# eridgd/WCT-TF

Hardware: AMD Instinct MI355X
Metric: stylized frames/sec @512x512, 5-level relu5->1 pipeline, alpha=0.8 (higher is better)
Workload: dtype f16

## Files before the change

### wct_tf_amd/build.py

```python
import hashlib
import os
import subprocess
import sys
from concurrent.futures import ThreadPoolExecutor

HERE = os.path.dirname(os.path.abspath(__file__))
CSRC = os.path.join(HERE, 'csrc')
LIB = os.path.join(HERE, 'libwct_hip.so')
WCT_UNITS = ['stats_gemm.hip', 'eigh.hip', 'spectral.hip', 'wct.hip', 'mask.hip', 'style_swap.hip', 'warm.hip']
API_UNITS = ['api_ctx.hip', 'api_weights.hip', 'api_drivers.hip', 'api_ops.hip', 'api_stylize.hip', 'api_train.hip']
SOURCES = API_UNITS + ['conv.hip', 'conv_wino.hip', 'coral.hip', 'colors.hip', 'noise.hip', 'banded.hip', 'train.hip'] + WCT_UNITS


STAMP = LIB + '.src.sha256'
FLAGS = ['--offload-arch=gfx950', '-O3', '-std=c++17', '-fPIC', '-Wno-unused-value', '-Wno-unused-result']
FILE_FLAGS = {u: ['-fno-slp-vectorize'] for u in WCT_UNITS}


def source_digest():
    h = hashlib.sha256((' '.join(FLAGS) + repr(sorted(FILE_FLAGS.items()))).encode())
    deps = sorted(os.path.join(CSRC, f) for f in os.listdir(CSRC) if f.endswith(('.hip', '.h')))
    deps.append(os.path.join(os.path.dirname(HERE), 'include', 'wct_hip.h'))
    for d in deps:
        h.update(os.path.basename(d).encode())
        h.update(open(d, 'rb').read())
    return h.hexdigest()


def needs_build():
    if not (os.path.exists(LIB) and os.path.exists(STAMP)):
        return True
    return open(STAMP).read().strip() != source_digest()


def build(force=False, verbose=True):
    if not force and not needs_build():
        return LIB
    hipcc = os.environ.get('HIPCC', '/opt/rocm/bin/hipcc')
    objs = [os.path.join(CSRC, src.replace('.hip', '.o')) for src in SOURCES]

    def compile_unit(src, obj):
        cmd = [hipcc] + FLAGS + FILE_FLAGS.get(src, []) + ['-c', os.path.join(CSRC, src), '-o', obj]
        if verbose:
            print(' '.join(cmd), flush=True)
        subprocess.check_call(cmd)

    with ThreadPoolExecutor(min(16, len(SOURCES))) as pool:
        list(pool.map(compile_unit, SOURCES, objs))
    cmd = [hipcc, '--offload-arch=gfx950', '-shared', '-fPIC', '-o', LIB] + objs
    if verbose:
        print(' '.join(cmd), flush=True)
    subprocess.check_call(cmd)
    with open(STAMP, 'w') as f:
        f.write(source_digest() + '\n')
    return LIB


if __name__ == '__main__':
    build(force='--force' in sys.argv)
    print(LIB)
```

### wct_tf_amd/csrc/spectral.hip

```cpp
#include "wct_stages.h"

__device__ __forceinline__ bool pair_resolved(float dp, float dq, float e) { return e * e <= 0.25f * dp * dq; }

constexpr float SPECTRAL_NOISE_CUT = 2.f;
__device__ __forceinline__ float spectral_cut(const float* Am, int C, int tid, float* red) {
  float mn = 0.f;
  for (int i = tid; i < C; i += 256) mn = fminf(mn, Am[(size_t)i * C + i]);
  for (int o = 32; o > 0; o >>= 1) mn = fminf(mn, __shfl_xor(mn, o, 64));
  if ((tid & 63) == 0) red[tid >> 6] = mn;
  __syncthreads();
  mn = fminf(fminf(red[0], red[1]), fminf(red[2], red[3]));
  return fmaxf(1e-5f, -SPECTRAL_NOISE_CUT * mn);
}

__device__ __forceinline__ float spectral_entry(float dp, float dq, float e, bool diag, int kind, float shift, float cut) {
  const bool kp = dp > cut, kq = dq > cut;
  if (diag) return kp ? (kind == 0 ? 1.f / sqrtf(dp + shift) : sqrtf(dp + shift)) : 0.f;
  if (!kp && !kq) return 0.f;
  if (kp && kq) {
    if (!pair_resolved(dp, dq, e)) return 0.f;
    const float sa = sqrtf(dp + shift), sb = sqrtf(dq + shift);
    return kind == 0 ? -e / (sa * sb * (sa + sb)) : e / (sa + sb);
  }
  const float dk = kp ? dp : dq, dd = kp ? dq : dp;
// ... 163 lines not shown
  spectral_tile_load(t, Am, C, p0, q0, tid);
  __syncthreads();
  const int ty = tid >> 4, tx = tid & 15;
#pragma unroll
  for (int i = 0; i < 4; ++i) {
    const int pl = ty * 4 + i, p = p0 + pl, q = q0 + tx * 4;
    if (p >= C || q >= C) continue;
    const f32x4 av = *reinterpret_cast<const f32x4*>(Am + (size_t)p * C + q);
    const float dp = t.dp[pl];
    f32x4 g, n4 = {0.f, 0.f, 0.f, 0.f}, r4 = n4, p4 = n4;
#pragma unroll
    for (int j = 0; j < 4; ++j) {
      const float dk = t.dq[tx * 4 + j];
      const float em = 0.5f * (av[j] + t.mt[tx * 4 + j][pl]);
      g[j] = spectral_entry(dp, dk, a.correct ? em : 0.f, p == q + j, kind, a.shift, cut);
      if (a.second && p != q + j && dp > cut && dk > cut && pair_resolved(dp, dk, em)) {
        const float sp = sqrtf(dp + a.shift), sk = sqrtf(dk + a.shift);
        n4[j] = em / (sp + sk);
        r4[j] = em / sk;
        p4[j] = n4[j] / sk;
      }
    }
    const size_t o = (size_t)p * C + q;
    *reinterpret_cast<f32x4*>(a.G + m * cc + o) = g;
    if (a.second) {
      *reinterpret_cast<f32x4*>(a.N + m * cc + o) = n4;
      if (kind == 0) { *reinterpret_cast<f32x4*>(a.R + pair * cc + o) = r4; *reinterpret_cast<f32x4*>(a.Pm + pair * cc + o) = p4; }
    }
  }
}

__global__ __launch_bounds__(256) void spectral_add2_all_kernel(SpecAllArgs a) {
  __shared__ float dps[64], dqs[64];
  __shared__ float x1t[64][65], x2t[64][65];
  const int m = blockIdx.z, p0 = blockIdx.y * 64, q0 = blockIdx.x * 64, tid = threadIdx.x;
  if (skip_style_mat(m, a.shared_style)) return;
  const int C = a.C, kind = m & 1;
  const size_t cc = (size_t)C * C;
  const float* Am = a.A + m * cc;
  float* Gm = a.G + m * cc;
  const float* X2 = a.X2 + m * cc;
  const float* X1 = a.X1 + (size_t)(m >> 1) * cc;
  int near = 0;
  for (int i = tid; i < C; i += 256) {
    const float d = fabsf(Am[(size_t)i * C + i]);
    near |= (d > 3.3e-6f) & (d < 3e-5f);
  }
  if (__syncthreads_or(near)) return;
  __shared__ float cutred[4];
  const float cut = spectral_cut(Am, C, tid, cutred);
  if (tid < 64) dps[tid] = p0 + tid < C ? Am[(size_t)(p0 + tid) * C + p0 + tid] : 0.f;
  else if (tid < 128) dqs[tid - 64] = q0 + tid - 64 < C ? Am[(size_t)(q0 + tid - 64) * C + q0 + tid - 64] : 0.f;
  const int ty = tid >> 4, tx = tid & 15;
#pragma unroll
  for (int i = 0; i < 4; ++i) {
    const int r = q0 + ty * 4 + i, c = p0 + tx * 4;
    f32x4 v1 = {0.f, 0.f, 0.f, 0.f}, v2 = v1;
    if (r < C && c < C) {
      v2 = *reinterpret_cast<const f32x4*>(X2 + (size_t)r * C + c);
      if (kind == 0) v1 = *reinterpret_cast<const f32x4*>(X1 + (size_t)r * C + c);
    }
#pragma unroll
    for (int j = 0; j < 4; ++j) { x2t[ty * 4 + i][tx * 4 + j] = v2[j]; x1t[ty * 4 + i][tx * 4 + j] = v1[j]; }
  }
  __syncthreads();
#pragma unroll
  for (int i = 0; i < 4; ++i) {
    const int pl = ty * 4 + i, p = p0 + pl, q = q0 + tx * 4;
    if (p >= C || q >= C) continue;
    const size_t o = (size_t)p * C + q;
    const f32x4 x2 = *reinterpret_cast<const f32x4*>(X2 + o);
    f32x4 x1 = {0.f, 0.f, 0.f, 0.f};
    if (kind == 0) x1 = *reinterpret_cast<const f32x4*>(X1 + o);
    f32x4 g = *reinterpret_cast<const f32x4*>(Gm + o);
    const float dp = dps[pl];
#pragma unroll
    for (int j = 0; j < 4; ++j) {
      const float dq = dqs[tx * 4 + j];
      if (!(dp > cut && dq > cut)) continue;
      const float sp = sqrtf(dp + a.shift), sq = sqrtf(dq + a.shift);
      float l2;
      if (kind == 1) l2 = -0.5f * (x2[j] + x2t[tx * 4 + j][pl]) / (sp + sq);
      else l2 = (0.5f * (x1[j] + x1t[tx * 4 + j][pl]) + 0.25f * (sp + sq) * (x2[j] + x2t[tx * 4 + j][pl])) / (sp * sq * (sp + sq));
      g[j] += l2;
    }
    *reinterpret_cast<f32x4*>(Gm + o) = g;
  }
}

int launch_spectral_function(const float* A, const float* V, float* G, float* X, float* out, int C, int nbatch,
                                    size_t stride, size_t out_stride, int kind, float shift, hipStream_t s, float* scratch2) {
  const size_t cc = (size_t)C * C;
  const dim3 tiles(cdiv(C, 64), cdiv(C, 64), nbatch);
  hipLaunchKernelGGL(spectral_matrix_kernel, tiles, dim3(256), 0, s, A, G, C, stride, kind, shift, EIG_CORRECT);
  HIP_TRY(hipGetLastError());
  if (scratch2 && EIG_CORRECT >= 2) {
    float* N = scratch2; float* R = N + nbatch * cc; float* Pm = R + nbatch * cc; float* X1 = Pm + nbatch * cc; float* X2 = X1 + nbatch * cc;
    hipLaunchKernelGGL(spectral_prep2_kernel, tiles, dim3(256), 0, s, A, N, R, Pm, C, stride, kind, shift);
    HIP_TRY(hipGetLastError());
    GemmArgs a = {};
    a.A = kind == 1 ? N : Pm; a.lda = C; a.a_kmajor = 0; a.B = N; a.ldb = C; a.b_kmajor = 1; a.sA = a.sB = cc;
    a.M = C; a.N = C; a.K = C; a.ksplit = C; a.out32 = X2; a.ldo = C; a.s_out = cc;
    int rc2 = launch_gemm(a, 1, nbatch, s);
    if (rc2) return rc2;
    if (kind == 0) {
      a.A = R; a.out32 = X1;
      if ((rc2 = launch_gemm(a, 1, nbatch, s))) return rc2;
    }
    hipLaunchKernelGGL(spectral_add2_kernel, tiles, dim3(256), 0, s, A, G, X1, X2, C, stride, kind, shift);
    HIP_TRY(hipGetLastError());
  }
  GemmArgs g = {};
  g.A = V; g.lda = C; g.a_kmajor = 0; g.B = G; g.ldb = C; g.b_kmajor = 1; g.sA = g.sB = stride;
  g.M = C; g.N = C; g.K = C; g.ksplit = C; g.out32 = X; g.ldo = C; g.s_out = stride;
  int rc = launch_gemm(g, 1, nbatch, s);
  if (rc) return rc;
  GemmArgs h = {};
  h.A = X; h.lda = C; h.a_kmajor = 0; h.B = V; h.ldb = C; h.b_kmajor = 0; h.sA = h.sB = stride;
  h.M = C; h.N = C; h.K = C; h.ksplit = C; h.out32 = out; h.ldo = C; h.s_out = out_stride;
  return launch_gemm(h, 1, nbatch, s);
}

int launch_refresh(const WctCarve& w, int C, int P, int shared_style, hipStream_t s, bool always) {
  const size_t cc = (size_t)C * C;
  int rc;
  GemmArgs r1 = {};
  r1.A = w.A0; r1.lda = C; r1.a_kmajor = 0; r1.B = w.V; r1.ldb = C; r1.b_kmajor = 1; r1.sA = r1.sB = cc; r1.skip_shared = shared_style;
  r1.M = C; r1.N = C; r1.K = C; r1.ksplit = C; r1.out32 = w.X; r1.ldo = C; r1.s_out = cc;
  if (!always) { r1.mask_diag = w.A; r1.s_mask = cc; r1.mask_out = w.refresh; }
  if ((rc = launch_gemm(r1, 1, 2 * P, s))) return rc;
  GemmArgs r2 = {};
  r2.A = w.V; r2.lda = C; r2.a_kmajor = 1; r2.B = w.X; r2.ldb = C; r2.b_kmajor = 1; r2.sA = r2.sB = cc; r2.skip_shared = shared_style;
  r2.M = C; r2.N = C; r2.K = C; r2.ksplit = C; r2.out32 = w.A; r2.ldo = C; r2.s_out = cc;
  if (!always) r2.mask_in = w.refresh;
  rc = launch_gemm(r2, 1, 2 * P, s);
  return rc;
}

int launch_spectral_tail(const WctCarve& w, int C, int P, float alpha, int mode, float eps_in, int shared_style, int nwhite,
                                hipStream_t s) {
  int rc;
  const size_t cc = (size_t)C * C;
  const float shift = mode == WCT_MODE_NP ? (eps_in >= 0.f ? eps_in : 1e-5f) : 0.f;
  const int second = EIG_CORRECT >= 2;
  const dim3 tiles(cdiv(C, 64), cdiv(C, 64), 2 * P);
  if ((rc = launch_refresh(w, C, P, shared_style, s))) return rc;
  SpecAllArgs sa = {};
  sa.A = w.A; sa.G = w.G; sa.C = C; sa.shift = shift; sa.correct = EIG_CORRECT; sa.second = second; sa.shared_style = shared_style;
  sa.N = w.S2; float* X2 = sa.N + 2 * P * cc; sa.R = X2 + 2 * P * cc; sa.Pm = sa.R + P * cc; float* X1 = sa.Pm + P * cc;
  sa.X1 = X1; sa.X2 = X2;
  sa.mabs = w.mabs; sa.mean = w.mean; sa.bias = w.bias; sa.alpha = alpha; sa.mode = mode;
  hipLaunchKernelGGL(spectral_open_all_kernel, tiles, dim3(256), 0, s, sa);
  HIP_TRY(hipGetLastError());
  if (second) {
    GemmArgs a = {};
    a.A = sa.Pm; a.sA = cc; a.A_odd = sa.N + cc; a.sA_odd = 2 * cc; a.lda = C; a.a_kmajor = 0;
    a.B = sa.N; a.ldb = C; a.b_kmajor = 1; a.sB = cc; a.skip_shared = shared_style;
    a.M = C; a.N = C; a.K = C; a.ksplit = C; a.out32 = X2; a.ldo = C; a.s_out = cc;
    if ((rc = launch_gemm(a, 1, 2 * P, s))) return rc;
    GemmArgs b = {};
    b.A = sa.R; b.sA = cc; b.lda = C; b.a_kmajor = 0; b.B = sa.N; b.ldb = C; b.b_kmajor = 1; b.sB = 2 * cc;
    b.M = C; b.N = C; b.K = C; b.ksplit = C; b.out32 = X1; b.ldo = C; b.s_out = cc;
    if (nwhite > 0 && (rc = launch_gemm(b, 1, nwhite, s))) return rc;
    hipLaunchKernelGGL(spectral_add2_all_kernel, tiles, dim3(256), 0, s, sa);
    HIP_TRY(hipGetLastError());
  }
  GemmArgs g = {};
  g.A = w.V; g.lda = C; g.a_kmajor = 0; g.B = w.G; g.ldb = C; g.b_kmajor = 1; g.sA = g.sB = cc; g.skip_shared = shared_style;
  g.M = C; g.N = C; g.K = C; g.ksplit = C; g.out32 = w.X; g.ldo = C; g.s_out = cc;
  if ((rc = launch_gemm(g, 1, 2 * P, s))) return rc;
  GemmArgs h = {};
  h.A = w.X; h.lda = C; h.a_kmajor = 0; h.B = w.V; h.ldb = C; h.b_kmajor = 0; h.sA = h.sB = cc; h.skip_shared = shared_style;
  h.M = C; h.N = C; h.K = C; h.ksplit = C; h.out32 = w.Tw; h.ldo = C; h.s_out = cc;
  if ((rc = launch_gemm(h, 1, 2 * P, s))) return rc;
  return WCT_OK;
}
```

### wct_tf_amd/csrc/wct.hip

```cpp
#include "wct_stages.h"
#include "jacobi_dev.h"
#include <algorithm>
#include <type_traits>



template <int BC, int BP, typename Args = ApplyArgs>
__global__ __launch_bounds__(256, 2) void apply_f16x2_kernel(Args p) {
  constexpr bool SEGB = std::is_same<Args, ApplySegBatchArgs>::value;
  constexpr bool SEG = std::is_same<Args, ApplySegArgs>::value || SEGB;
  constexpr int TM = BC / 64, TN = BP / 64;
  constexpr int MI = BC * 4 / 256, XI = BP * 4 / 256;
  __shared__ __attribute__((aligned(16))) unsigned char lm[2][BC * 64];
  __shared__ __attribute__((aligned(16))) unsigned char lx[2][BP * 64];
  typedef unsigned int u32x4 __attribute__((ext_vector_type(4)));
  const int tid = threadIdx.x, lane = tid & 63, wave = tid >> 6;
  const int wm = wave >> 1, wn = wave & 1;
  const int pair = blockIdx.z;
  const int n0 = blockIdx.x * BP, c0 = blockIdx.y * BC;
  int seg0 = 0, N = p.N;
  [[maybe_unused]] int row0 = 0;
  if constexpr (SEGB) {
    const int f = seg_frame(p.fl[pair]), lab = seg_label(p.fl[pair]);
    const int first = p.seg_off[f * (WCT_MIX_MAX + 1) + lab];
// ... 77 lines not shown
#pragma unroll
    for (int ks = 0; ks < 2; ++ks) {
      const int chunk = ks * 2 + (lane >> 5);
      half8 ah[TM], al[TM], bh[TN], bl[TN];
#pragma unroll
      for (int i = 0; i < TM; ++i) {
        const int r = (wm * TM + i) * 32 + (lane & 31);
        const int off = (r * 4 + (chunk ^ ((r >> 2) & 3))) * 16;
        ah[i] = *reinterpret_cast<const half8*>(lm[0] + off);
        al[i] = *reinterpret_cast<const half8*>(lm[1] + off);
      }
#pragma unroll
      for (int j = 0; j < TN; ++j) {
        const int r = (wn * TN + j) * 32 + (lane & 31);
        const int off = (r * 4 + (chunk ^ ((r >> 2) & 3))) * 16;
        bh[j] = *reinterpret_cast<const half8*>(lx[0] + off);
        bl[j] = *reinterpret_cast<const half8*>(lx[1] + off);
      }
#pragma unroll
      for (int i = 0; i < TM; ++i)
#pragma unroll
        for (int j = 0; j < TN; ++j) {
          acc[i][j] = __builtin_amdgcn_mfma_f32_32x32x16_f16(al[i], bh[j], acc[i][j], 0, 0, 0);
          acc[i][j] = __builtin_amdgcn_mfma_f32_32x32x16_f16(ah[i], bl[j], acc[i][j], 0, 0, 0);
          acc[i][j] = __builtin_amdgcn_mfma_f32_32x32x16_f16(ah[i], bh[j], acc[i][j], 0, 0, 0);
        }
    }
    __syncthreads();
  }

  const float inv = 1.f / (sx * sM);
  const float* bias = p.bias + (size_t)pair * C;
  const int kgrp = lane >> 5;
  f32x4 bvs[TM][4];
#pragma unroll
  for (int i = 0; i < TM; ++i)
#pragma unroll
    for (int rq = 0; rq < 4; ++rq) {
      const int co = c0 + (wm * TM + i) * 32 + 8 * rq + 4 * kgrp;
      const f32x4 z = {0.f, 0.f, 0.f, 0.f};
      bvs[i][rq] = co < C ? *reinterpret_cast<const f32x4*>(bias + co) : z;
    }
  int dst[TN];
  if constexpr (SEG)
#pragma unroll
    for (int j = 0; j < TN; ++j) {
      const int n = n0 + (wn * TN + j) * 32 + (lane & 31);
      dst[j] = p.perm[seg0 + (n < N ? n : 0)];
      if constexpr (SEGB) dst[j] += row0;
    }
#pragma unroll
  for (int j = 0; j < TN; ++j) {
    const int n = n0 + (wn * TN + j) * 32 + (lane & 31);
    const bool n_ok = n < N;
    const size_t row = SEG ? (size_t)dst[j] * C : ((size_t)pair * N + (n_ok ? n : 0)) * C;
#pragma unroll
    for (int i = 0; i < TM; ++i) {
      const int cb = c0 + (wm * TM + i) * 32;
      unsigned pk[4][2];
#pragma unroll
      for (int rq = 0; rq < 4; ++rq) {
        const int co = cb + 8 * rq + 4 * kgrp;
        const f32x4 bv = bvs[i][rq];
        f32x4 v;
#pragma unroll
        for (int q = 0; q < 4; ++q) v[q] = acc[i][j][rq * 4 + q] * inv + bv[q];
        if (p.out32 && n_ok && co < C) *reinterpret_cast<f32x4*>(p.out32 + row + co) = v;
        typedef _Float16 h2 __attribute__((ext_vector_type(2)));
        h2 lo = {(half_t)v[0], (half_t)v[1]}, hi = {(half_t)v[2], (half_t)v[3]};
        pk[rq][0] = __builtin_bit_cast(unsigned, lo);
        pk[rq][1] = __builtin_bit_cast(unsigned, hi);
      }
      if (p.out16) {
#pragma unroll
        for (int m = 0; m < 2; ++m) {
          auto sxw = __builtin_amdgcn_permlane32_swap(pk[2 * m][0], pk[2 * m + 1][0], false, false);
          auto syw = __builtin_amdgcn_permlane32_swap(pk[2 * m][1], pk[2 * m + 1][1], false, false);
          u32x4 o = {sxw[0], syw[0], sxw[1], syw[1]};
          const int co = cb + 16 * m + 8 * kgrp;
          if (n_ok && co < C) *reinterpret_cast<u32x4*>(p.out16 + row + co) = o;
        }
      }
    }
  }
}

int launch_apply_seg(const ApplySegArgs& a, int nmax, int P, hipStream_t s) {
  const int C = a.C;
  if (C >= 128) hipLaunchKernelGGL((apply_f16x2_kernel<128, 128, ApplySegArgs>), dim3(cdiv(nmax, 128), cdiv(C, 128), P), dim3(256), 0, s, a);
  else hipLaunchKernelGGL((apply_f16x2_kernel<64, 128, ApplySegArgs>), dim3(cdiv(nmax, 128), cdiv(C, 64), P), dim3(256), 0, s, a);
  HIP_TRY(hipGetLastError());
  return WCT_OK;
}

int launch_apply_seg_batch(const ApplySegBatchArgs& a, int nmax, int P, hipStream_t s) {
  const int C = a.C;
  if (C >= 128) hipLaunchKernelGGL((apply_f16x2_kernel<128, 128, ApplySegBatchArgs>), dim3(cdiv(nmax, 128), cdiv(C, 128), P), dim3(256), 0, s, a);
  else hipLaunchKernelGGL((apply_f16x2_kernel<64, 128, ApplySegBatchArgs>), dim3(cdiv(nmax, 128), cdiv(C, 64), P), dim3(256), 0, s, a);
  HIP_TRY(hipGetLastError());
  return WCT_OK;
}

static int wct_nslab(int N) { int s = cdiv(N, 64); return s < 1 ? 1 : (s > 256 ? 256 : s); }

static void cov_split(int C, int Nmax, int P, int* nsplit, int* ksplit) {
  const int nt = C >= 128 ? cdiv(C, 128) : 1;
  const int tiles = nt * (nt + 1) / 2 * P;
  int want = 32 / tiles;
  if (want < 1) want = 1;
  int ks = cdiv(cdiv(Nmax, want), 32) * 32;
  if (ks < 256) ks = 256;
  *ksplit = ks;
  *nsplit = cdiv(Nmax, ks);
}

PairLayout pair_layout(int C, int Nc, int Ns) {
  PairLayout L;
  const int Nmax = Nc > Ns ? Nc : Ns;
  L.nslab = wct_nslab(Nmax);
  cov_split(C, Nmax, 1, &L.nsplit, &L.ksplit);
  return L;
}

WctCarve carve(void* base, int C, int P, const PairLayout& lay) {
  WctCarve w;
  w.nslab = lay.nslab; w.nsplit = lay.nsplit; w.ksplit = lay.ksplit;
  size_t off = 0;
  char* b = reinterpret_cast<char*>(base);
  auto take = [&](size_t bytes) { void* p = b ? b + off : nullptr; off += align_up(bytes); return p; };
  const size_t cc = (size_t)C * C * sizeof(float);
  w.mean = (float*)take((size_t)2 * P * C * sizeof(float));
  w.var = (float*)take((size_t)2 * P * C * sizeof(float));
  w.stat_partial = (float*)take((size_t)2 * P * w.nslab * C * sizeof(float));
  w.absmax = (float*)take((size_t)2 * P * w.nslab * sizeof(float));
  w.scale = (float*)take((size_t)2 * P * sizeof(float));
  w.cov_partial = (float*)take((size_t)2 * P * w.nsplit * cc);
  w.A = (float*)take(2 * P * cc);
  w.A0 = (float*)take(2 * P * cc);
  w.refresh = (int*)take((size_t)2 * P * sizeof(int));
  w.V = (float*)take(2 * P * cc);
  w.d = (float*)take((size_t)2 * P * C * sizeof(float));
  w.G = (float*)take(2 * P * cc);
  w.X = (float*)take(2 * P * cc);
  w.S2 = (float*)take(7 * P * cc);
  w.Tw = (float*)take(2 * P * cc);
  w.Tcs = w.Tw + (size_t)C * C;
  w.T = (float*)take(P * cc);
  w.M = (float*)take(P * cc);
  w.bias = (float*)take((size_t)P * C * sizeof(float));
  w.mabs = (unsigned*)take((size_t)P * sizeof(unsigned));
  w.jacobi_bytes = jacobi_workspace_bytes(C, 2 * P) + 4 * (1024 + 64 * sizeof(JacobiState));
  w.jacobi_ws = take(w.jacobi_bytes);
  w.mix = (float*)take((size_t)2 * C * sizeof(float));
  w.total = off;
  return w;
}

size_t wct_workspace_bytes(int C, int Nc, int Ns, int P) {
  const int Cw = C < 32 ? 32 : C;
  return carve(nullptr, Cw, P, pair_layout(Cw, Nc, Ns)).total;
}

int launch_blend(const WctCarve& w, int C, int P, float alpha, int shared_style, hipStream_t s) {
  const size_t cc = (size_t)C * C;
  GemmArgs g = {};
  g.A = w.Tcs; g.lda = C; g.a_kmajor = 0; g.B = w.Tw; g.ldb = C; g.b_kmajor = 1; g.sA = shared_style ? 0 : 2 * cc; g.sB = 2 * cc;
  g.M = C; g.N = C; g.K = C; g.ksplit = C; g.out32 = w.M; g.ldo = C; g.s_out = cc;
  g.blend = 1; g.alpha = alpha; g.mabs = w.mabs;
  return launch_gemm(g, 1, P, s);
}

int launch_apply(const WctCarve& w, const float* content, int Nc, int C, int P, half_t* out16, float* out32, hipStream_t s) {
  ApplyArgs a;
  a.x = content; a.N = Nc; a.C = C; a.mean = w.mean; a.M = w.M; a.bias = w.bias;
  a.xscale = w.scale; a.mabs = w.mabs; a.out16 = out16; a.out32 = out32;
  if (C >= 128) hipLaunchKernelGGL((apply_f16x2_kernel<128, 128>), dim3(cdiv(Nc, 128), cdiv(C, 128), P), dim3(256), 0, s, a);
  else hipLaunchKernelGGL((apply_f16x2_kernel<64, 128>), dim3(cdiv(Nc, 128), cdiv(C, 64), P), dim3(256), 0, s, a);
  HIP_TRY(hipGetLastError());
  return WCT_OK;
}

static int launch_blend_apply(const WctCarve& w, const float* content, int Nc, int C, int P, float alpha, int shared_style,
                              half_t* out16, float* out32, hipStream_t s) {
  int rc;
  if ((rc = launch_blend(w, C, P, alpha, shared_style, s))) return rc;
  return launch_apply(w, content, Nc, C, P, out16, out32, s);
}

WctStyleKey wct_style_key(int C, int Nc, int Ns) {
  const PairLayout L = pair_layout(std::max(C, 32), Nc, Ns);
  return WctStyleKey{L.nslab, L.nsplit, L.ksplit};
}
size_t wct_style_state_floats(int C) { return (size_t)2 * C + (size_t)C * C; }

template <typename Ref>
__global__ __launch_bounds__(256) void style_load_kernel(Ref r, float* mean, float* var, float* Tw, int C, int with_T) {
  const int k = blockIdx.y;
  const float* src = r.state[k];
  const size_t cc = (size_t)C * C, n = (size_t)2 * C + (with_T ? cc : 0), slot = (size_t)(2 * k + 1);
  for (size_t i = (blockIdx.x * (size_t)blockDim.x + threadIdx.x) * 4; i < n; i += (size_t)gridDim.x * blockDim.x * 4) {
    const f32x4 v = *reinterpret_cast<const f32x4*>(src + i);
    float* dst = i < (size_t)C ? mean + slot * C + i : (i < (size_t)2 * C ? var + slot * C + (i - C) : Tw + slot * cc + (i - 2 * C));
    *reinterpret_cast<f32x4*>(dst) = v;
  }
}

static int launch_style_load(const WctStyleRef& r, int K, const WctCarve& w, int C, bool with_T, hipStream_t s) {
  for (int k = 0; k < K; ++k) ARG_CHECK(r.state[k] != nullptr);
  const size_t n4 = ((size_t)2 * C + (with_T ? (size_t)C * C : 0)) / 4;
  hipLaunchKernelGGL(style_load_kernel<WctStyleRef>, dim3((unsigned)std::min<size_t>((n4 + 255) / 256, 256), K), dim3(256), 0, s, r, w.mean,
                     w.var, w.Tw, C, with_T ? 1 : 0);
  HIP_TRY(hipGetLastError());
  return WCT_OK;
}

int launch_style_load_slots(const WctStyleSlots& r, int P, const WctCarve& w, int C, bool with_T, hipStream_t s) {
  ARG_CHECK(P >= 1 && P <= WCT_PLAN_PAIRS);
  for (int p = 0; p < P; ++p) ARG_CHECK(r.state[p] != nullptr);
  const size_t n4 = ((size_t)2 * C + (with_T ? (size_t)C * C : 0)) / 4;
  hipLaunchKernelGGL(style_load_kernel<WctStyleSlots>, dim3((unsigned)std::min<size_t>((n4 + 255) / 256, 256), P), dim3(256), 0, s, r, w.mean,
                     w.var, w.Tw, C, with_T ? 1 : 0);
  HIP_TRY(hipGetLastError());
  return WCT_OK;
}

static void style_plan(SlotPlan* sp, void* base, int C, const float* style, int Ns, const WctStyleKey& key) {
  *sp = SlotPlan{};
  sp->P = 1; sp->skip = WCT_SKIP_CONTENT; sp->nwhite = 0;
  sp->slot[1] = {style, Ns, PairLayout{key.nslab, key.nsplit, key.ksplit}};
  plan_carve(sp, base, C);
}

size_t wct_style_workspace_bytes(int C, int Ns, const WctStyleKey& key) {
  SlotPlan sp;
  style_plan(&sp, nullptr, C, nullptr, Ns, key);
  return sp.total;
}

int launch_style_state(const float* style, int Ns, int C, const WctStyleKey& key, int adain, int mode, float eps_in, void* workspace,
                       size_t workspace_bytes, int* eig_fail, hipStream_t s, float* state) {
  ARG_CHECK(style && state && C % 32 == 0 && C >= 32 && C <= 1024 && Ns >= (adain ? 1 : 2) && launch_map_fits((size_t)Ns * C, 4));
  ARG_CHECK(adain || mode == WCT_MODE_NP || mode == WCT_MODE_TF);
  ARG_CHECK(key.nslab >= 1 && key.nslab <= 256 && key.nsplit >= 1 && key.ksplit >= 256 && key.ksplit % 32 == 0 &&
            (long long)key.nsplit * key.ksplit >= Ns);
  SlotPlan sp;
  style_plan(&sp, workspace, C, style, Ns, key);
  ARG_CHECK(workspace_bytes >= sp.total);
  const WctCarve& w = sp.w;
  int rc;
  if (adain) {
    if ((rc = launch_plan_stats(sp, C, true, false, 0.f, s))) return rc;
    HIP_TRY(hipMemcpyAsync(state + C, w.var + C, (size_t)C * sizeof(float), hipMemcpyDeviceToDevice, s));
  } else {
    if ((rc = launch_plan_stats(sp, C, false, true, cov_eps(mode, eps_in), s))) return rc;
    if ((rc = launch_eig_stage(w, C, sp.P, sp.skip, 1, nullptr, eig_fail, s))) return rc;
    if ((rc = launch_spectral_tail(w, C, sp.P, 1.f, mode, eps_in, sp.skip, sp.nwhite, s))) return rc;
    HIP_TRY(hipMemcpyAsync(state + 2 * C, w.Tw + (size_t)C * C, (size_t)C * C * sizeof(float), hipMemcpyDeviceToDevice, s));
  }
  HIP_TRY(hipMemcpyAsync(state, w.mean + C, (size_t)C * sizeof(float), hipMemcpyDeviceToDevice, s));
  return WCT_OK;
}

int launch_wct(const float* content, int Nc, const float* style, int Ns, int C, int P, float alpha, int mode, float eps_in,
               half_t* out16, float* out32, void* workspace, size_t workspace_bytes, int* sweeps_dev,
               int stages, hipStream_t s, int shared_style, int* eig_fail, const WctFeatStats* stats, const WctStyleRef* prep,
               const WctWarmRef* warm) {
  ARG_CHECK(C % 32 == 0 && C >= 32 && C <= 1024 && Nc >= 2 && Ns >= 2 && P >= 1 && P <= 32);
  ARG_CHECK(!warm || (warm->basis && (shared_style == 0 || prep)));
  if (prep) shared_style = WCT_SKIP_STYLE;
  ARG_CHECK(mode == WCT_MODE_NP || mode == WCT_MODE_TF);
  ARG_CHECK(launch_map_fits((size_t)Nc * C, 4) && launch_map_fits((size_t)Ns * C, 4));
  WctCarve w = carve(workspace, C, P, pair_layout(C, Nc, Ns));
  ARG_CHECK(workspace_bytes >= w.total);
  int rc;
  if (stages & WCT_STAGE_COV) {
    if ((rc = launch_means(content, Nc, style, Ns, C, P, w, false, shared_style, s, stats))) return rc;
    if ((rc = launch_cov(content, Nc, style, Ns, C, P, w, cov_eps(mode, eps_in), shared_style, s))) return rc;
  }
  if (stages & WCT_STAGE_EIG) {
    const bool rotate = warm && warm->valid;
    if (rotate && (rc = launch_warm_rotate(w, C, P, warm->basis, s))) return rc;
    if ((rc = launch_eig_stage(w, C, P, shared_style, (stages & WCT_STAGE_EIG_FP32UPDATE) ? 0 : 1, sweeps_dev, eig_fail, s, rotate ? 0 : 2)))
      return rc;
    if (rotate && (rc = launch_warm_compose(w, C, P, warm->basis, s))) return rc;
    if (warm && (rc = launch_warm_store(w.V + (size_t)2 * (P - 1) * C * C, w.X, warm->basis, C, s))) return rc;
  }
  if (!(stages & WCT_STAGE_APPLY)) return WCT_OK;

  if (prep && (rc = launch_style_load(*prep, 1, w, C, true, s))) return rc;
  if ((rc = launch_spectral_tail(w, C, P, alpha, mode, eps_in, shared_style, P, s))) return rc;
  return launch_blend_apply(w, content, Nc, C, P, alpha, shared_style, out16, out32, s);
}

void plan_carve(SlotPlan* sp, void* base, int C) {
  PairLayout mx = {1, 1, 0};
  for (int m = 0; m < 2 * sp->P; ++m)
    if (sp->slot[m].n) { mx.nslab = std::max(mx.nslab, sp->slot[m].lay.nslab); mx.nsplit = std::max(mx.nsplit, sp->slot[m].lay.nsplit); }
  sp->w = carve(base, C, std::max(sp->P, 1), mx);
  sp->total = sp->w.total;
}

bool plan_fits(const SlotPlan& sp, int C) {
  for (int m = 0; m < 2 * sp.P; ++m)
    if (!launch_map_fits((size_t)sp.slot[m].n * C, 4)) return false;
  return true;
}

static bool mix_plan(SlotPlan* sp, void* base, int C, const float* content, int Nc, const float* const* styles, const int* Ns,
                     int K, const float* lambda, int nmin, const WctFeatStats* stats, bool prepared = false) {
  if (!Ns || !lambda || K < 1 || K > WCT_MIX_MAX) return false;
  int ref = 0;
  for (int k = 0; k < K; ++k) {
    if ((styles && !styles[k]) || Ns[k] < nmin || !(lambda[k] >= 0.f && lambda[k] <= 1.f)) return false;
    if (lambda[k] > lambda[ref]) ref = k;
  }
  const int Cw = std::max(C, 32);
// ... 147 lines not shown
```

### wct_tf_amd/csrc/wct_stages.h

```cpp
#pragma once
#include "common.h"

constexpr int WCT_SKIP_MIX = 2;
constexpr int WCT_SKIP_STYLE = 3, WCT_SKIP_CONTENT = 4, WCT_SKIP_MIX_STYLE = 5;
constexpr int WCT_SKIP_STYLES = 6;
__device__ __host__ __forceinline__ bool skip_style_mat(int mat, int shared_style) {
  if (shared_style >= WCT_SKIP_STYLE)
    return shared_style == WCT_SKIP_STYLE ? (mat & 1) != 0
                                          : (shared_style == WCT_SKIP_CONTENT ? (mat & 1) == 0
                                                                              : (shared_style == WCT_SKIP_MIX_STYLE ? mat > 0 : (mat & 1) != 0));
  return shared_style == WCT_SKIP_MIX ? ((mat & 1) == 0 && mat > 0) : (shared_style && (mat & 1) && mat > 1);
}
__device__ __host__ __forceinline__ bool one_content(int shared_style) { return shared_style == WCT_SKIP_MIX || shared_style == WCT_SKIP_MIX_STYLE; }
__device__ __host__ __forceinline__ bool one_style(int shared_style) { return shared_style == 1 || shared_style == WCT_SKIP_STYLE; }

constexpr int EIG_CORRECT = 2;
constexpr float JACOBI_TOL_FN = 1.5e-2f;
constexpr float JACOBI_TOL_FN2 = 4e-2f;
constexpr float JACOBI_TOL_FN_WCT = EIG_CORRECT >= 2 ? JACOBI_TOL_FN2 : (EIG_CORRECT ? JACOBI_TOL_FN : 0.f);

static inline size_t align_up(size_t x) { return (x + 255) & ~(size_t)255; }

struct WctCarve {
  float *mean, *var, *stat_partial, *absmax, *scale, *cov_partial, *A, *A0, *V, *d, *G, *X, *S2, *Tw, *Tcs, *T, *M, *bias, *mix;
  unsigned* mabs; int* refresh;
  void* jacobi_ws; size_t jacobi_bytes;
  int nslab, nsplit, ksplit;
  size_t total;
};

struct PairLayout { int nslab, nsplit, ksplit; };
PairLayout pair_layout(int C, int Nc, int Ns);
WctCarve carve(void* base, int C, int P, const PairLayout& lay);

static inline float cov_eps(int mode, float eps_in) {
  return mode == WCT_MODE_TF ? (eps_in >= 0.f ? eps_in : 1e-8f) : 0.f;
}

static inline unsigned rows_grid(size_t N, int C) {
  const size_t blocks = (N * C / 4 + 255) / 256;
  return (unsigned)(blocks > 2048 ? 2048 : blocks);
}

constexpr int WCT_PLAN_PAIRS = 32;
struct SlotPlan {
  int P, skip, nwhite;
  struct Slot { const float* x; int n; PairLayout lay; } slot[2 * WCT_PLAN_PAIRS];
  const float* u0; const unsigned* umax0;
  WctCarve w;
  size_t total;
};
void plan_carve(SlotPlan* sp, void* base, int C);
bool plan_fits(const SlotPlan& sp, int C);

struct ApplyArgs {
  const float* x; int N; int C;
  const float* mean;
  const float* M; const float* bias;
  const float* xscale;
  const unsigned* mabs;
  half_t* out16; float* out32;
};
struct ApplySegArgs : ApplyArgs { const int* seg_off; const int* perm; int lab[WCT_MIX_MAX]; };
struct ApplySegBatchArgs : ApplyArgs { const int* seg_off; const int* perm; unsigned char fl[WCT_PLAN_PAIRS]; };
__device__ __host__ __forceinline__ int seg_frame(unsigned char fl) { return fl >> 3; }
__device__ __host__ __forceinline__ int seg_label(unsigned char fl) { return fl & 7; }

int launch_means(const float* content, int Nc, const float* style, int Ns, int C, int P, const WctCarve& w, bool with_var,
                 int shared_style, hipStream_t s, const WctFeatStats* fs = nullptr);
int launch_cov(const float* content, int Nc, const float* style, int Ns, int C, int P, const WctCarve& w, float eps, int shared_style,
               hipStream_t s);
int launch_plan_stats(const SlotPlan& sp, int C, bool with_var, bool with_cov, float eps, hipStream_t s);
int launch_eig_stage(const WctCarve& w, int C, int P, int skip, int u_f16, int* sweeps_dev, int* eig_fail, hipStream_t s,
                     int check_from = 2);
int launch_refresh(const WctCarve& w, int C, int P, int shared_style, hipStream_t s, bool always = false);
int launch_spectral_tail(const WctCarve& w, int C, int P, float alpha, int mode, float eps_in, int shared_style, int nwhite, hipStream_t s);
int launch_spectral_function(const float* A, const float* V, float* G, float* X, float* out, int C, int nbatch, size_t stride,
                             size_t out_stride, int kind, float shift, hipStream_t s, float* scratch2 = nullptr);
int launch_blend(const WctCarve& w, int C, int P, float alpha, int shared_style, hipStream_t s);
int launch_apply(const WctCarve& w, const float* content, int Nc, int C, int P, half_t* out16, float* out32, hipStream_t s);
int launch_apply_seg(const ApplySegArgs& a, int nmax, int P, hipStream_t s);
int launch_apply_seg_batch(const ApplySegBatchArgs& a, int nmax, int P, hipStream_t s);
int launch_warm_rotate(const WctCarve& w, int C, int P, const float* V0, hipStream_t s);
int launch_warm_compose(const WctCarve& w, int C, int P, const float* V0, hipStream_t s);
int launch_warm_store(const float* V, float* scratch, float* basis, int C, hipStream_t s);
int launch_style_load_slots(const WctStyleSlots& r, int P, const WctCarve& w, int C, bool with_T, hipStream_t s);
```

Measured before the change: 680.9.

## Use split-f16 MFMA GEMMs for spectral and blend stages at large C

For C>=256, the CxC fp32 GEMMs in the spectral tail (second-order correction, V·G·V^T) and in the blend are replaced by a split-plane scheme. Each operand is scaled per row and split into hi and lo f16 planes, then multiplied with three f16 MFMA products (hi*hi plus the two cross terms), which approximates fp32 accuracy on matrix cores. The aim is to swap the slower fp32 GEMM path for f16 tensor-core throughput. The cost is extra split kernels, added workspace, and slightly reduced precision compared with true fp32.

```diff
diff --git a/wct_tf_amd/build.py b/wct_tf_amd/build.py
--- a/wct_tf_amd/build.py
+++ b/wct_tf_amd/build.py
@@ -7,7 +7,7 @@
 HERE = os.path.dirname(os.path.abspath(__file__))
 CSRC = os.path.join(HERE, 'csrc')
 LIB = os.path.join(HERE, 'libwct_hip.so')
-WCT_UNITS = ['stats_gemm.hip', 'eigh.hip', 'spectral.hip', 'wct.hip', 'mask.hip', 'style_swap.hip', 'warm.hip']
+WCT_UNITS = ['stats_gemm.hip', 'eigh.hip', 'spectral.hip', 'spectral_gemm.hip', 'wct.hip', 'mask.hip', 'style_swap.hip', 'warm.hip']
 API_UNITS = ['api_ctx.hip', 'api_weights.hip', 'api_drivers.hip', 'api_ops.hip', 'api_stylize.hip', 'api_train.hip']
 SOURCES = API_UNITS + ['conv.hip', 'conv_wino.hip', 'coral.hip', 'colors.hip', 'noise.hip', 'banded.hip', 'train.hip'] + WCT_UNITS
 
diff --git a/wct_tf_amd/csrc/spectral.hip b/wct_tf_amd/csrc/spectral.hip
--- a/wct_tf_amd/csrc/spectral.hip
+++ b/wct_tf_amd/csrc/spectral.hip
@@ -339,7 +339,12 @@
   sa.mabs = w.mabs; sa.mean = w.mean; sa.bias = w.bias; sa.alpha = alpha; sa.mode = mode;
   hipLaunchKernelGGL(spectral_open_all_kernel, tiles, dim3(256), 0, s, sa);
   HIP_TRY(hipGetLastError());
-  if (second) {
+  const bool f16 = C >= SPLIT_GEMM_MIN_C;
+  if (second && f16) {
+    if ((rc = launch_spectral_second_f16(w, C, P, shared_style, nwhite, sa.N, sa.Pm, sa.R, X2, X1, s))) return rc;
+    hipLaunchKernelGGL(spectral_add2_all_kernel, tiles, dim3(256), 0, s, sa);
+    HIP_TRY(hipGetLastError());
+  } else if (second) {
     GemmArgs a = {};
     a.A = sa.Pm; a.sA = cc; a.A_odd = sa.N + cc; a.sA_odd = 2 * cc; a.lda = C; a.a_kmajor = 0;
     a.B = sa.N; a.ldb = C; a.b_kmajor = 1; a.sB = cc; a.skip_shared = shared_style;
@@ -352,6 +357,7 @@
     hipLaunchKernelGGL(spectral_add2_all_kernel, tiles, dim3(256), 0, s, sa);
     HIP_TRY(hipGetLastError());
   }
+  if (f16) return launch_spectral_vgvt_f16(w, C, P, shared_style, s);
   GemmArgs g = {};
   g.A = w.V; g.lda = C; g.a_kmajor = 0; g.B = w.G; g.ldb = C; g.b_kmajor = 1; g.sA = g.sB = cc; g.skip_shared = shared_style;
   g.M = C; g.N = C; g.K = C; g.ksplit = C; g.out32 = w.X; g.ldo = C; g.s_out = cc;
diff --git a/wct_tf_amd/csrc/spectral_gemm.hip b/wct_tf_amd/csrc/spectral_gemm.hip
--- /dev/null
+++ b/wct_tf_amd/csrc/spectral_gemm.hip
@@ -0,0 +1,298 @@
+#include "wct_stages.h"
+
+struct SplitArgs {
+  const float* src; size_t s_src;
+  half_t* planes; float* inv;
+  int C, transpose, skip_shared;
+};
+
+constexpr float LO_UP = 2048.f, LO_DOWN = 1.f / 2048.f;
+
+__device__ __forceinline__ float split_scale(float m) {
+  if (!(m > 0.f && m < 1e30f)) return 1.f;
+  int e;
+  frexpf(m, &e);
+  return ldexpf(1.f, min(14 - e, 96));
+}
+
+__global__ __launch_bounds__(256) void split_planes_kernel(SplitArgs a) {
+  __shared__ float red[8][32];
+  __shared__ float tt[32][33];
+  const int b = blockIdx.y, x0 = blockIdx.x * 32, tid = threadIdx.x, C = a.C;
+  if (a.skip_shared && skip_style_mat(b, a.skip_shared)) return;
+  const size_t cc = (size_t)C * C;
+  const float* S = a.src + b * a.s_src;
+  half_t* hi = a.planes + (size_t)b * 2 * cc;
+  half_t* lo = hi + cc;
+  const int xr = tid >> 3, kq = tid & 7;
+  float m = 0.f;
+  if (!a.transpose) {
+    const float* row = S + (size_t)(x0 + xr) * C + kq * 4;
+#pragma unroll 4
+    for (int k0 = 0; k0 < C; k0 += 32) {
+      const f32x4 v = *reinterpret_cast<const f32x4*>(row + k0);
+      m = fmaxf(fmaxf(m, fmaxf(fabsf(v[0]), fabsf(v[1]))), fmaxf(fabsf(v[2]), fabsf(v[3])));
+    }
+    for (int o = 1; o < 8; o <<= 1) m = fmaxf(m, __shfl_xor(m, o, 64));
+  } else {
+    const int col = tid & 31, rg = tid >> 5;
+#pragma unroll 4
+    for (int k = rg; k < C; k += 8) m = fmaxf(m, fabsf(S[(size_t)k * C + x0 + col]));
+    red[rg][col] = m;
+    __syncthreads();
+    m = 0.f;
+#pragma unroll
+    for (int g = 0; g < 8; ++g) m = fmaxf(m, red[g][xr]);
+  }
+  const float sc = split_scale(m);
+  if (kq == 0) a.inv[(size_t)b * C + x0 + xr] = 1.f / sc;
+  auto put = [&](const f32x4& v, int k0) {
+    half4 h, l;
+#pragma unroll
+    for (int j = 0; j < 4; ++j) {
+      const float t = v[j] * sc;
+      h[j] = (half_t)t;
+      l[j] = (half_t)((t - (float)h[j]) * LO_UP);
+    }
+    const size_t o = (size_t)(x0 + xr) * C + k0 + kq * 4;
+    *reinterpret_cast<half4*>(hi + o) = h;
+    *reinterpret_cast<half4*>(lo + o) = l;
+  };
+  if (!a.transpose) {
+    const float* row = S + (size_t)(x0 + xr) * C + kq * 4;
+#pragma unroll 4
+    for (int k0 = 0; k0 < C; k0 += 32) put(*reinterpret_cast<const f32x4*>(row + k0), k0);
+  } else {
+    const int col = tid & 31, rg = tid >> 5;
+    const float* src = S + (size_t)rg * C + x0 + col;
+    float nx[4];
+#pragma unroll
+    for (int i = 0; i < 4; ++i) nx[i] = src[(size_t)(8 * i) * C];
+    for (int k0 = 0; k0 < C; k0 += 32) {
+      __syncthreads();
+#pragma unroll
+      for (int i = 0; i < 4; ++i) tt[rg + 8 * i][col] = nx[i];
+      __syncthreads();
+      if (k0 + 32 < C)
+#pragma unroll
+        for (int i = 0; i < 4; ++i) nx[i] = src[(size_t)(k0 + 32 + 8 * i) * C];
+      f32x4 v;
+#pragma unroll
+      for (int j = 0; j < 4; ++j) v[j] = tt[kq * 4 + j][xr];
+      put(v, k0);
+    }
+  }
+}
+
+static int launch_split(const WctCarve& w, int first, const float* src, size_t s_src, int C, int nbatch, int transpose, hipStream_t s,
+                        int skip_shared = 0) {
+  if (nbatch <= 0) return WCT_OK;
+  SplitArgs a;
+  a.src = src; a.s_src = s_src; a.planes = w.planes + (size_t)first * 2 * C * C; a.inv = w.pinv + (size_t)first * C;
+  a.C = C; a.transpose = transpose; a.skip_shared = skip_shared;
+  hipLaunchKernelGGL(split_planes_kernel, dim3(C / 32, nbatch), dim3(256), 0, s, a);
+  HIP_TRY(hipGetLastError());
+  return WCT_OK;
+}
+
+struct PlaneGemmArgs {
+  const half_t* planes; const float* inv;
+  int a0, sa, a_odd, sa_odd, b0, sb;
+  int C, nbatch;
+  float* out; size_t s_out;
+  int skip_shared;
+  int blend; float alpha; unsigned* mabs;
+};
+
+template <int BT>
+__global__ __launch_bounds__(256, 2) void plane_gemm_kernel(PlaneGemmArgs p) {
+  constexpr int TM = BT / 64;
+  constexpr int PI = BT * 4 / 256;
+  __shared__ __attribute__((aligned(16))) unsigned char lds[2][4][BT * 64];
+  const int tid = threadIdx.x, lane = tid & 63, wave = tid >> 6;
+  const int wm = wave >> 1, wn = wave & 1;
+  const int C = p.C;
+  const int nt = (C + BT - 1) / BT, T = nt * nt;
+  int batch, tile;
+  {
+    const int L = blockIdx.x, full = (p.nbatch >> 3) * 8 * T;
+    if (L < full) { const int r = L % (8 * T); batch = (L / (8 * T)) * 8 + (r & 7); tile = r >> 3; }
+    else { batch = (p.nbatch >> 3) * 8 + (L - full) / T; tile = (L - full) % T; }
+  }
+  const int m0 = (tile / nt) * BT, n0 = (tile % nt) * BT;
+  if (p.skip_shared && skip_style_mat(batch, p.skip_shared)) return;
+  const size_t cc = (size_t)C * C;
+  const int ib = p.b0 + batch * p.sb;
+  const int ia = p.a_odd >= 0 ? ((batch & 1) ? p.a_odd + (batch >> 1) * p.sa_odd : p.a0 + (batch >> 1) * p.sa) : p.a0 + batch * p.sa;
+  const half_t* Ah = p.planes + (size_t)ia * 2 * cc;
+  const half_t* Bh = p.planes + (size_t)ib * 2 * cc;
+
+  const half_t *pa[PI], *pb[PI];
+  int off[PI];
+#pragma unroll
+  for (int i = 0; i < PI; ++i) {
+    const int item = tid + i * 256, row = item >> 2, kq = item & 3;
+    pa[i] = Ah + (size_t)min(m0 + row, C - 1) * C + kq * 8;
+    pb[i] = Bh + (size_t)min(n0 + row, C - 1) * C + kq * 8;
+    off[i] = (row * 4 + (kq ^ ((row >> 2) & 3))) * 16;
+  }
+
+  f32x16 acc[TM][TM], acx[TM][TM];
+#pragma unroll
+  for (int i = 0; i < TM; ++i)
+#pragma unroll
+    for (int j = 0; j < TM; ++j)
+#pragma unroll
+      for (int r = 0; r < 16; ++r) { acc[i][j][r] = 0.f; acx[i][j][r] = 0.f; }
+
+  half8 ra[PI][2], rb[PI][2];
+  auto load = [&](int k0) {
+#pragma unroll
+    for (int i = 0; i < PI; ++i) {
+      ra[i][0] = *reinterpret_cast<const half8*>(pa[i] + k0);
+      ra[i][1] = *reinterpret_cast<const half8*>(pa[i] + cc + k0);
+      rb[i][0] = *reinterpret_cast<const half8*>(pb[i] + k0);
+      rb[i][1] = *reinterpret_cast<const half8*>(pb[i] + cc + k0);
+    }
+  };
+
+  auto store = [&](int buf) {
+#pragma unroll
+    for (int i = 0; i < PI; ++i) {
+      *reinterpret_cast<half8*>(lds[buf][0] + off[i]) = ra[i][0];
+      *reinterpret_cast<half8*>(lds[buf][1] + off[i]) = ra[i][1];
+      *reinterpret_cast<half8*>(lds[buf][2] + off[i]) = rb[i][0];
+      *reinterpret_cast<half8*>(lds[buf][3] + off[i]) = rb[i][1];
+    }
+  };
+
+  load(0);
+  store(0);
+  if (32 < C) load(32);
+  for (int k0 = 0, cur = 0; k0 < C; k0 += 32, cur ^= 1) {
+    __syncthreads();
+#pragma unroll
+    for (int ks = 0; ks < 2; ++ks) {
+      const int chunk = ks * 2 + (lane >> 5);
+      half8 ah[TM], al[TM], bh[TM], bl[TM];
+#pragma unroll
+      for (int i = 0; i < TM; ++i) {
+        const int r = (wm * TM + i) * 32 + (lane & 31);
+        const int o = (r * 4 + (chunk ^ ((r >> 2) & 3))) * 16;
+        ah[i] = *reinterpret_cast<const half8*>(lds[cur][0] + o);
+        al[i] = *reinterpret_cast<const half8*>(lds[cur][1] + o);
+      }
+#pragma unroll
+      for (int j = 0; j < TM; ++j) {
+        const int r = (wn * TM + j) * 32 + (lane & 31);
+        const int o = (r * 4 + (chunk ^ ((r >> 2) & 3))) * 16;
+        bh[j] = *reinterpret_cast<const half8*>(lds[cur][2] + o);
+        bl[j] = *reinterpret_cast<const half8*>(lds[cur][3] + o);
+      }
+#pragma unroll
+      for (int i = 0; i < TM; ++i)
+#pragma unroll
+        for (int j = 0; j < TM; ++j) {
+          acx[i][j] = __builtin_amdgcn_mfma_f32_32x32x16_f16(al[i], bh[j], acx[i][j], 0, 0, 0);
+          acx[i][j] = __builtin_amdgcn_mfma_f32_32x32x16_f16(ah[i], bl[j], acx[i][j], 0, 0, 0);
+          acc[i][j] = __builtin_amdgcn_mfma_f32_32x32x16_f16(ah[i], bh[j], acc[i][j], 0, 0, 0);
+        }
+    }
+    if (k0 + 32 < C) {
+      store(cur ^ 1);
+      if (k0 + 64 < C) load(k0 + 64);
+    }
+  }
+
+  const float* inva = p.inv + (size_t)ia * C;
+  const float* invb = p.inv + (size_t)ib * C;
+  f32x4 sa4[TM][4];
+  float sbv[TM];
+#pragma unroll
+  for (int i = 0; i < TM; ++i)
+#pragma unroll
+    for (int rq = 0; rq < 4; ++rq) {
+      const int gm = m0 + (wm * TM + i) * 32 + 8 * rq + 4 * (lane >> 5);
+      sa4[i][rq] = *reinterpret_cast<const f32x4*>(inva + min(gm, C - 4));
+    }
+#pragma unroll
+  for (int j = 0; j < TM; ++j) sbv[j] = invb[min(n0 + (wn * TM + j) * 32 + (lane & 31), C - 1)];
+#pragma unroll
+  for (int j = 0; j < TM; ++j) asm volatile("" : "+v"(sbv[j]));
+  float* out = p.out + batch * p.s_out;
+  float av = 0.f;
+#pragma unroll
+  for (int i = 0; i < TM; ++i)
+#pragma unroll
+    for (int j = 0; j < TM; ++j) {
+      const int gn = n0 + (wn * TM + j) * 32 + (lane & 31);
+#pragma unroll
+      for (int r = 0; r < 16; ++r) {
+        const int gm = m0 + (wm * TM + i) * 32 + (r & 3) + 8 * (r >> 2) + 4 * (lane >> 5);
+        if (gm < C && gn < C) {
+          float v = (acc[i][j][r] + acx[i][j][r] * LO_DOWN) * sa4[i][r >> 2][r & 3] * sbv[j];
+          if (p.blend) {
+            v = p.alpha * v;
+            if (gm == gn) v += 1.f - p.alpha;
+            av = fmaxf(av, fabsf(v));
+          }
+          out[(size_t)gm * C + gn] = v;
+        }
+      }
+    }
+  if (p.blend) {
+    for (int o = 32; o > 0; o >>= 1) av = fmaxf(av, __shfl_xor(av, o, 64));
+    if (lane == 0 && av < 1e30f) atomicMax(p.mabs + batch, __float_as_uint(av));
+  }
+}
+
+static int launch_plane_gemm(PlaneGemmArgs g, const WctCarve& w, int C, int nbatch, hipStream_t s) {
+  if (nbatch <= 0) return WCT_OK;
+  g.planes = w.planes; g.inv = w.pinv; g.C = C; g.nbatch = nbatch;
+  const bool small_grid = (long)cdiv(C, 128) * cdiv(C, 128) * nbatch < 256;
+  if (!small_grid) hipLaunchKernelGGL((plane_gemm_kernel<128>), dim3(cdiv(C, 128) * cdiv(C, 128) * nbatch), dim3(256), 0, s, g);
+  else hipLaunchKernelGGL((plane_gemm_kernel<64>), dim3(cdiv(C, 64) * cdiv(C, 64) * nbatch), dim3(256), 0, s, g);
+  HIP_TRY(hipGetLastError());
+  return WCT_OK;
+}
+
+
+int launch_spectral_second_f16(const WctCarve& w, int C, int P, int shared_style, int nwhite, const float* N, const float* Pm,
+                               const float* R, float* X2, float* X1, hipStream_t s) {
+  const size_t cc = (size_t)C * C;
+  int rc;
+  if ((rc = launch_split(w, 0, N, cc, C, 2 * P, 0, s, shared_style))) return rc;
+  if ((rc = launch_split(w, 2 * P, Pm, cc, C, nwhite, 0, s))) return rc;
+  if ((rc = launch_split(w, 3 * P, R, cc, C, nwhite, 0, s))) return rc;
+  PlaneGemmArgs a = {};
+  a.a0 = 2 * P; a.sa = 1; a.a_odd = 1; a.sa_odd = 2; a.b0 = 0; a.sb = 1; a.out = X2; a.s_out = cc; a.skip_shared = shared_style;
+  if ((rc = launch_plane_gemm(a, w, C, 2 * P, s))) return rc;
+  PlaneGemmArgs b = {};
+  b.a0 = 3 * P; b.sa = 1; b.a_odd = -1; b.b0 = 0; b.sb = 2; b.out = X1; b.s_out = cc;
+  return launch_plane_gemm(b, w, C, nwhite, s);
+}
+
+int launch_spectral_vgvt_f16(const WctCarve& w, int C, int P, int shared_style, hipStream_t s) {
+  const size_t cc = (size_t)C * C;
+  int rc;
+  if ((rc = launch_split(w, 0, w.V, cc, C, 2 * P, 0, s, shared_style))) return rc;
+  if ((rc = launch_split(w, 2 * P, w.G, cc, C, 2 * P, 1, s, shared_style))) return rc;
+  PlaneGemmArgs g = {};
+  g.a0 = 0; g.sa = 1; g.a_odd = -1; g.b0 = 2 * P; g.sb = 1; g.out = w.X; g.s_out = cc; g.skip_shared = shared_style;
+  if ((rc = launch_plane_gemm(g, w, C, 2 * P, s))) return rc;
+  if ((rc = launch_split(w, 2 * P, w.X, cc, C, 2 * P, 0, s, shared_style))) return rc;
+  PlaneGemmArgs h = {};
+  h.a0 = 2 * P; h.sa = 1; h.a_odd = -1; h.b0 = 0; h.sb = 1; h.out = w.Tw; h.s_out = cc; h.skip_shared = shared_style;
+  return launch_plane_gemm(h, w, C, 2 * P, s);
+}
+
+int launch_blend_f16(const WctCarve& w, int C, int P, float alpha, int one_tcs, hipStream_t s) {
+  const size_t cc = (size_t)C * C;
+  int rc;
+  if ((rc = launch_split(w, 0, w.Tcs, 2 * cc, C, one_tcs ? 1 : P, 0, s))) return rc;
+  if ((rc = launch_split(w, P, w.Tw, 2 * cc, C, P, 1, s))) return rc;
+  PlaneGemmArgs g = {};
+  g.a0 = 0; g.sa = one_tcs ? 0 : 1; g.a_odd = -1; g.b0 = P; g.sb = 1; g.out = w.M; g.s_out = cc;
+  g.blend = 1; g.alpha = alpha; g.mabs = w.mabs;
+  return launch_plane_gemm(g, w, C, P, s);
+}
diff --git a/wct_tf_amd/csrc/wct.hip b/wct_tf_amd/csrc/wct.hip
--- a/wct_tf_amd/csrc/wct.hip
+++ b/wct_tf_amd/csrc/wct.hip
@@ -253,6 +253,9 @@
   w.jacobi_bytes = jacobi_workspace_bytes(C, 2 * P) + 4 * (1024 + 64 * sizeof(JacobiState));
   w.jacobi_ws = take(w.jacobi_bytes);
   w.mix = (float*)take((size_t)2 * C * sizeof(float));
+  const int nsets = C >= SPLIT_GEMM_MIN_C ? 4 * P : 0;
+  w.planes = (half_t*)take((size_t)nsets * cc);
+  w.pinv = (float*)take((size_t)nsets * C * sizeof(float));
   w.total = off;
   return w;
 }
@@ -263,6 +266,7 @@
 }
 
 int launch_blend(const WctCarve& w, int C, int P, float alpha, int shared_style, hipStream_t s) {
+  if (C >= SPLIT_GEMM_MIN_C) return launch_blend_f16(w, C, P, alpha, shared_style ? 1 : 0, s);
   const size_t cc = (size_t)C * C;
   GemmArgs g = {};
   g.A = w.Tcs; g.lda = C; g.a_kmajor = 0; g.B = w.Tw; g.ldb = C; g.b_kmajor = 1; g.sA = shared_style ? 0 : 2 * cc; g.sB = 2 * cc;
diff --git a/wct_tf_amd/csrc/wct_stages.h b/wct_tf_amd/csrc/wct_stages.h
--- a/wct_tf_amd/csrc/wct_stages.h
+++ b/wct_tf_amd/csrc/wct_stages.h
@@ -24,6 +24,7 @@
 struct WctCarve {
   float *mean, *var, *stat_partial, *absmax, *scale, *cov_partial, *A, *A0, *V, *d, *G, *X, *S2, *Tw, *Tcs, *T, *M, *bias, *mix;
   unsigned* mabs; int* refresh;
+  half_t* planes; float* pinv;
   void* jacobi_ws; size_t jacobi_bytes;
   int nslab, nsplit, ksplit;
   size_t total;
@@ -77,6 +78,11 @@
 int launch_spectral_tail(const WctCarve& w, int C, int P, float alpha, int mode, float eps_in, int shared_style, int nwhite, hipStream_t s);
 int launch_spectral_function(const float* A, const float* V, float* G, float* X, float* out, int C, int nbatch, size_t stride,
                              size_t out_stride, int kind, float shift, hipStream_t s, float* scratch2 = nullptr);
+constexpr int SPLIT_GEMM_MIN_C = 256;
+int launch_spectral_second_f16(const WctCarve& w, int C, int P, int shared_style, int nwhite, const float* N, const float* Pm,
+                               const float* R, float* X2, float* X1, hipStream_t s);
+int launch_spectral_vgvt_f16(const WctCarve& w, int C, int P, int shared_style, hipStream_t s);
+int launch_blend_f16(const WctCarve& w, int C, int P, float alpha, int one_tcs, hipStream_t s);
 int launch_blend(const WctCarve& w, int C, int P, float alpha, int shared_style, hipStream_t s);
 int launch_apply(const WctCarve& w, const float* content, int Nc, int C, int P, half_t* out16, float* out32, hipStream_t s);
 int launch_apply_seg(const ApplySegArgs& a, int nmax, int P, hipStream_t s);
```

Measured after the change: 686.9 (median of 6 runs). Within noise of the previous version (+0.9%).
